# rjagerman/pytorchltr

Hardware: AMD Instinct MI355X
Metric: queries/sec loss fwd+bwd (B=1024, list_len=128) + achieved HBM GB/s (higher is better)
Workload: dtype f32; 1 GPU; c2: Linear(136,1) scorer + hinge loss fwd+bwd, B=1024/GPU, list_len=128, n~U[1,128]; global_batch=1024, list_len=128, features=136, loss=hinge, mode=eager, parallelism=dp1, batches_in_rotation=5, repeats=1, statistic=one timed region of --steps steps after --warmup steps

## Files before the change

### include/ltr_sched.h

```cpp
#ifndef LTR_SCHED_H
#define LTR_SCHED_H

#include "ltr_hip.h"

#ifdef __cplusplus
extern "C" {
#endif

LTR_DEBUG_HOOK int ltr_debug_sched_slots(int B, int G, int cus, int nred, int *group, int *rank);
LTR_DEBUG_HOOK int ltr_debug_lazy_holdback(int packed);

#ifdef __cplusplus
}
#endif

#endif
```

### pytorchltr_amd/_C.py

```python
import ctypes
import os

import torch

_HERE = os.path.dirname(os.path.abspath(__file__))
LIB_PATH = os.environ.get("LTR_HIP_LIB") or os.path.join(_HERE, "csrc", "libltr_hip.so")

HINGE, DCG_HINGE, LOGISTIC, ARP1, ARP2, NDCG1, NDCG2 = range(7)
LABEL_I64, LABEL_F32, LABEL_I32 = 0, 1, 2
ERR_CONFIG = -6
ERR_TIMEOUT = -7
PLAN_NONE, PLAN_REGISTER_TILE, PLAN_CLUSTER, PLAN_GENERAL, PLAN_PARTS = 0, 1, 2, 3, 4

_vp, _i, _f, _sz = ctypes.c_void_p, ctypes.c_int, ctypes.c_float, ctypes.c_size_t

SIGNATURES = {
    "ltr_version": (_i, []),
    "ltr_error_string": (ctypes.c_char_p, [_i]),
    "ltr_max_list_len": (_i, []),
    "ltr_max_list_len_f64": (_i, []),
    "ltr_device_status": (_i, [_i]),
    "ltr_debug_force_timeout": (None, [_i]),
    "ltr_debug_cluster_mode": (None, [_i]),
    "ltr_debug_parts_all": (_i, [_i]),
# ... 53 lines not shown
    "ltr_linear_lazy_rows_reduce_f32": (_i, [_i, _i, _i, _i, _f, _vp, _i, _vp, _vp, _vp, _i, _vp]),
    "ltr_debug_fake_allreduce": (_i, [_vp, _vp, _sz, _i, _i, _vp, _vp]),
    "ltr_mailbox_create": (_i, [_i, _i, _i, _vp, _vp]),
    "ltr_mailbox_connect": (_i, [_vp, _vp]),
    "ltr_mailbox_destroy": (_i, [_vp]),
    "ltr_mailbox_allreduce": (_i, [_vp, _vp, _sz, _i, _i, _vp, _vp]),
    "ltr_debug_mailbox_state": (_i, [_vp, ctypes.c_longlong, ctypes.c_longlong]),
    "ltr_mailbox_set_timeout_ms": (ctypes.c_longlong, [ctypes.c_longlong]),
    "ltr_linear_pairwise_f32": (_i, [_i, _f, _vp, _vp, _vp, _vp, _i, _vp, _vp, _i, _i, _i,
                                     _vp, _vp, _vp, _vp, _vp, _sz, _vp]),
    "ltr_linear_partials_f32": (_i, [_i, _f, _vp, _vp, _vp, _vp, _i, _vp, _i, _i, _i,
                                     _vp, _vp, _vp, _vp]),
    "ltr_linear_reduce_f32": (_i, [_vp, _vp, _i, _i, _vp, _vp, _vp]),
    "ltr_linear_reduce_bcast_f32": (_i, [_vp, _vp, _i, _i, _vp, _vp, _vp]),
    "ltr_linear_reduce_loss_f32": (_i, [_vp, _vp, _vp, _i, _i, _vp, _vp, _vp, _vp]),
    "ltr_linear_reduce_accum_f32": (_i, [_vp, _vp, _vp, _i, _i, _vp, _vp, _vp, _i, _vp]),
    "ltr_linear_scores_f32": (_i, [_vp, _vp, _vp, _vp, _i, _i, _i, _vp, _vp]),
    "ltr_linear_grad_workspace_bytes": (_sz, [_i, _i, _i]),
    "ltr_linear_grad_f32": (_i, [_vp, _vp, _vp, _i, _i, _i, _vp, _vp, _sz, _vp]),
    "ltr_mlp_max_list_len": (_i, [_i]),
    "ltr_mlp_param_count": (_sz, [_i, _i, _i]),
    "ltr_mlp_workspace_bytes": (_sz, [_i, _i, _i, _i]),
    "ltr_mlp_scores_f32": (_i, [_vp, _vp, _vp, _vp, _vp, _vp, _vp, _vp, _i, _i, _i, _i, _i, _vp, _vp]),
    "ltr_mlp_pairwise_f32": (_i, [_i, _f, _vp, _vp, _vp, _vp, _vp, _vp, _vp, _vp, _i, _vp, _vp,
                                  _i, _i, _i, _i, _i, _vp, _vp, _vp, _vp, _vp, _sz, _vp]),
}

EVAL_SIGNATURES = {
    "ltr_eval_workspace_bytes": (_sz, [_i, _i, _vp, _i]),
    "ltr_eval_f32": (_i, [_vp, _vp, _i, _vp, _vp, _i, ctypes.c_uint64, _vp, _i, _i, _vp, _i, _f, _i, _f, _vp, _vp,
                          _sz, _vp]),
}

LISTWISE_LISTNET, LISTWISE_LISTMLE = 0, 1

LISTWISE_SIGNATURES = {
    "ltr_listmle_workspace_bytes": (_sz, [_i, _i]),
    "ltr_listmle_f32": (_i, [_vp, _vp, _i, _vp, _i, _vp, _i, ctypes.c_uint64, _vp, _i, _i, _vp, _vp, _vp, _sz, _vp]),
    "ltr_linear_listwise_plan": (_i, [_i, _i, _i, _i]),
    "ltr_linear_listwise_partials_f32": (_i, [_i, _i, _vp, _vp, _vp, _vp, _i, _vp, _vp, _i, ctypes.c_uint64, _vp, _i, _i, _i,
                                              _vp, _vp, _vp, _vp]),
    "ltr_mlp_listwise_plan": (_i, [_i, _i, _i, _i, _i, _i]),
    "ltr_mlp_listwise_f32": (_i, [_i, _i] + [_vp] * 7 + [_vp, _i, _vp, _vp, _i, ctypes.c_uint64, _vp, _vp]
                             + [_i] * 5 + [_vp] * 5 + [_sz, _vp]),
}

MLP_ROWS_SIGNATURES = {
    "ltr_mlp_rows_scores_f32": (_i, [_vp] * 8 + [_i] * 5 + [_vp, _vp]),
    "ltr_mlp_rows_grad_workspace_bytes": (_sz, [_i, _i, _i, _i, _i]),
    "ltr_mlp_rows_grad_f32": (_i, [_vp] * 9 + [_i] * 5 + [_vp, _vp, _sz, _vp]),
}

MLP_BF16_SIGNATURES = {
    "ltr_mlp_bf16_scores": (_i, [_vp] * 8 + [_i] * 5 + [_vp, _vp]),
    "ltr_mlp_bf16_grad_workspace_bytes": (_sz, [_i, _i, _i, _i, _i]),
    "ltr_mlp_bf16_grad": (_i, [_vp] * 9 + [_i] * 5 + [_vp, _vp, _sz, _vp]),
}

LINEAR_BF16_SIGNATURES = {
    "ltr_linear_scores_bf16": (_i, [_vp, _vp, _vp, _vp, _i, _i, _i, _vp, _vp]),
    "ltr_linear_grad_workspace_bytes_bf16": (_sz, [_i, _i, _i]),
    "ltr_linear_grad_bf16": (_i, [_vp, _vp, _vp, _i, _i, _i, _vp, _vp, _sz, _vp]),
    "ltr_linear_bf16_plan": (_i, [_i, _i, _i, _i]),
    "ltr_linear_partials_bf16": (_i, [_i, _f, _vp, _vp, _vp, _vp, _i, _vp, _i, _i, _i, _vp, _vp, _vp, _vp]),
    "ltr_collate_pad_bf16": (_i, [_vp, _vp, _vp, _vp, _vp, _i, _i, _i, _i, _vp, _vp, _vp, _vp]),
}

MLP_WIDE_SIGNATURES = {
    "ltr_mlp_wide_scores_f32": (_i, [_vp] * 8 + [_i] * 5 + [_vp, _vp]),
    "ltr_mlp_wide_grad_workspace_bytes": (_sz, [_i, _i, _i, _i, _i]),
    "ltr_mlp_wide_grad_f32": (_i, [_vp] * 9 + [_i] * 5 + [_vp, _vp, _sz, _vp]),
}

LONGPAIR_SIGNATURES = {
    "ltr_max_pair_list_len": (_i, []),
    "ltr_long_pair_geometry": (None, [_vp, _vp]),
    "ltr_pairwise_loss_long_workspace_bytes": (_sz, [_i, _i, _i]),
    "ltr_pairwise_loss_long_f32": (_i, [_i, _f, _vp, _vp, _i, _vp, _i, _i, _vp, _vp, _vp, _sz, _vp]),
    "ltr_debug_long_pairs_all": (_i, [_i]),
}

SCHED_SIGNATURES = {
    "ltr_debug_sched_slots": (_i, [_i, _i, _i, _i, _vp, _vp]),
    "ltr_debug_lazy_holdback": (_i, [_i]),
}

_lib = None


class ExtensionMissingError(ImportError):
    pass


class _Library(ctypes.CDLL):

    def __getattr__(self, name):
        try:
            return super().__getattr__(name)
        except AttributeError:
            if name.startswith("ltr_debug_"):
                raise AttributeError(
                    "%s is a test / tuning hook and this libltr_hip.so was built without them (LTR_NO_DEBUG_HOOKS=1); "
                    "rebuild with `python -m pytorchltr_amd.build --force` and the variable unset" % name) from None
            raise


def lib():
    global _lib
    if _lib is None:
        if not os.path.exists(LIB_PATH):
            raise ExtensionMissingError(
                "pytorchltr_amd HIP extension not found at %s; build it with "
                "`python -m pytorchltr_amd.build` (hipcc --offload-arch=gfx950). "
                "There is no CPU fallback." % LIB_PATH)
        handle = _Library(LIB_PATH)
        for name, (restype, argtypes) in (list(SIGNATURES.items()) + list(EVAL_SIGNATURES.items())
                                          + list(LISTWISE_SIGNATURES.items()) + list(LONGPAIR_SIGNATURES.items())
                                          + list(MLP_ROWS_SIGNATURES.items()) + list(MLP_WIDE_SIGNATURES.items())
                                          + list(MLP_BF16_SIGNATURES.items()) + list(LINEAR_BF16_SIGNATURES.items())
                                          + list(SCHED_SIGNATURES.items())):
            if name.startswith("ltr_debug_") and not hasattr(handle, name):
                continue
            fn = getattr(handle, name)
            fn.restype = restype
            fn.argtypes = argtypes
        _lib = handle
    return _lib


def check(rc):
    if rc != 0:
        msg = lib().ltr_error_string(int(rc))
        raise RuntimeError("pytorchltr_amd: %s (code %d)" % (msg.decode() if msg else "?", rc))


def ptr(t):
    return None if t is None else t.data_ptr()


try:
    _raw_stream = torch._C._cuda_getCurrentRawStream
except AttributeError:
    _raw_stream = None


def stream_of(t):
    if _raw_stream is not None:
        return _raw_stream(t.device.index if t.device.index is not None else torch.cuda.current_device())
    return torch.cuda.current_stream(t.device).cuda_stream


class _NullCtx:
    def __enter__(self):
        return self

    def __exit__(self, *exc):
        return False


_NULL = _NullCtx()


def device_ctx(t):
    idx = t.device.index
    if idx is None or idx == torch.cuda.current_device():
        return _NULL
# ... 78 lines not shown
```

### pytorchltr_amd/csrc/ltr_common.inc

```
#pragma once
#include <hip/hip_runtime.h>
#include <hip/hip_ext.h>
#include <stdint.h>
#include <stdio.h>
#include <stdlib.h>
#include <type_traits>

#include "ltr_hip.h"

extern "C" __attribute__((visibility("hidden"))) int *ltr_internal_status_device_ptr(void *stream);
extern "C" __attribute__((visibility("hidden"))) int ltr_internal_status_peek(void);
extern "C" __attribute__((visibility("hidden"))) void ltr_internal_exchange_mark_dirty(void);

namespace {

constexpr int kWave = 64;
constexpr int kMaxListLen = 4096;
constexpr int kSymMaxLen = 1024;
constexpr int kLossSymMaxLen = 2048;
constexpr float kLog2e = 1.4426950408889634f;
constexpr float kLn2 = 0.6931471805599453f;

#define LTR_CLEAR_STALE_ERROR() ((void)hipGetLastError())

// ... 25 lines not shown
    if (dtype == LTR_LABEL_I64)
        stage_rows_t(sy, srow, (const int64_t *)rel + row, L, nb, tid, T);
    else if (dtype == LTR_LABEL_F32)
        stage_rows_t(sy, srow, (const float *)rel + row, L, nb, tid, T);
    else
        stage_rows_t(sy, srow, (const int32_t *)rel + row, L, nb, tid, T);
}

template <typename LabelT>
__device__ __forceinline__ void stage_labels_t(float2 *sy, const LabelT *__restrict__ yrow, int L,
                                               int nb, int tid, int T)
{
    for (int m = tid; m < L; m += T) {
        const float yv = (float)yrow[m];
        if (m < nb) sy[m].y = yv;
    }
}

__device__ __forceinline__ void stage_labels(float2 *sy, const void *rel, int dtype, size_t row,
                                             int L, int nb, int tid, int T)
{
    if (dtype == LTR_LABEL_I64) stage_labels_t(sy, (const int64_t *)rel + row, L, nb, tid, T);
    else if (dtype == LTR_LABEL_F32) stage_labels_t(sy, (const float *)rel + row, L, nb, tid, T);
    else stage_labels_t(sy, (const int32_t *)rel + row, L, nb, tid, T);
}

__device__ __forceinline__ int clamp_n(int64_t n, int L)
{
    return n < 0 ? 0 : (n > (int64_t)L ? L : (int)n);
}

constexpr int kSchedMaxPerCu = 4;
constexpr int kLossSchedMaxPerCu = 16;
constexpr int kSchedLowBits = 3;

struct SchedSlot { int group, rank; };
__host__ __device__ inline int sched_round(int id, int cus, int &r)
{
    int t = 0;
    r = id;
    if (r >= 4 * cus) { r -= 4 * cus; t += 4; }
    if (r >= 2 * cus) { r -= 2 * cus; t += 2; }
    if (r >= cus) { r -= cus; t += 1; }
    return t;
}
__host__ __device__ inline bool sched_quiet(int id, int cus, int nred)
{
    if (nred <= 0 || nred >= cus || id < cus) return false;
    int r;
    sched_round(id, cus, r);
    return r < nred;
}
__host__ __device__ inline SchedSlot sched_slot(int id, int B, int G, int cus, int nred)
{
    int pos = id - nred;
    if (nred > 0 && nred < cus) {
        int r, re;
        const int t = sched_round(id, cus, r);
        const int below = t > 0 ? (t - 1) * nred + (r < nred ? r : nred) : 0;
        if (t > 0 && r < nred) {
            const int te = sched_round(nred + B, cus, re);
            const int Q = te > 0 ? (te - 1) * nred + (re < nred ? re : nred) : 0;
            pos = B - Q + below;
        } else {
            pos -= below;
        }
    }
    const int u = pos >> 3;
    int jp = u / G;
    SchedSlot s;
    s.group = u - jp * G;
    if (cus > 0) {
        const int per = cus / (8 * G);
        if (per >= 2) {
            const int rd = jp / per, base = rd * per;
            const int back = (rd ^ (rd >> 1)) & 1;
            if (back && (base + per) * 8 * G <= B) jp = base + (per - 1 - (jp - base));
        }
    }
    s.rank = jp * 8 + (pos & 7);
    return s;
}

__device__ __forceinline__ int sched_query_sampled(const int64_t *__restrict__ n, int B, int L, int G, int tid,
                                                   int &nb_out, int pos, int round_cus = 0, int nred = 0)
{
    __shared__ int s_sel[2];
    if (tid < 64) {
        const int lane = tid;
        const SchedSlot slot = sched_slot(pos, B, G, round_cus, nred);
        const int gam = slot.group;
        int rho = slot.rank;
        const int id = ((lane >> 3) * G + gam) * 8 + (lane & 7);
        unsigned long long cand = __ballot(id < B);
        const int key = clamp_n(n[min(id, B - 1)], L);
        const bool flat = __ballot(key != __builtin_amdgcn_readfirstlane(key)) == 0ull;
        for (int bt = flat ? -1 : 31 - __builtin_clz(L); bt >= kSchedLowBits; --bt) {
            const unsigned long long m = __ballot(((key >> bt) & 1) != 0) & cand;
            const int c = __popcll(m);
            if (rho < c) cand = m;
            else { rho -= c; cand &= ~m; }
        }
        const int below = __popcll(cand & ((1ull << lane) - 1ull));
        if ((((cand >> lane) & 1ull) != 0ull) && below == rho) { s_sel[0] = id; s_sel[1] = key; }
    }
    __syncthreads();
    nb_out = __builtin_amdgcn_readfirstlane(s_sel[1]);
    return __builtin_amdgcn_readfirstlane(s_sel[0]);
}

template <int CTRL, int ROW_MASK>
__device__ __forceinline__ float dpp_move(float v)
{
    return __int_as_float(__builtin_amdgcn_update_dpp(0, __float_as_int(v), CTRL, ROW_MASK, 0xF, false));
}

__device__ __forceinline__ float quad_sum(float v)
{
    v += dpp_move<0xB1, 0xF>(v);
    v += dpp_move<0x4E, 0xF>(v);
    return v;
}

__device__ __forceinline__ float wave_sum(float v)
{
    v = quad_sum(v);
    v += dpp_move<0x141, 0xF>(v);
    v += dpp_move<0x140, 0xF>(v);
    v += dpp_move<0x142, 0xA>(v);
    v += dpp_move<0x143, 0xC>(v);
    return __int_as_float(__builtin_amdgcn_readlane(__float_as_int(v), 63));
}

__device__ __forceinline__ void lds_barrier()
{
    asm volatile("s_waitcnt lgkmcnt(0)\n\ts_barrier" ::: "memory");
}

__device__ __forceinline__ float block_sum(float v, float *red)
{
    v = wave_sum(v);
    const int nw = blockDim.x >> 6;
    if (nw == 1) return v;
    __syncthreads();
    if ((threadIdx.x & 63) == 0) red[threadIdx.x >> 6] = v;
    __syncthreads();
    float t = 0.f;
    for (int i = 0; i < nw; ++i) t += red[i];
    return t;
}

struct OpAdd { static constexpr float id = 0.f; static __device__ __forceinline__ float f(float a, float b) { return a + b; } };
struct OpMul { static constexpr float id = 1.f; static __device__ __forceinline__ float f(float a, float b) { return a * b; } };
struct OpMin { static constexpr float id = 3.0e38f; static __device__ __forceinline__ float f(float a, float b) { return fminf(a, b); } };

template <typename Op>
__device__ __forceinline__ float block_reduce(float v, float *red)
{
#pragma unroll
    for (int o = 32; o > 0; o >>= 1) v = Op::f(v, __shfl_xor(v, o, kWave));
    const int nw = blockDim.x >> 6;
    if (nw == 1) return v;
    __syncthreads();
    if ((threadIdx.x & 63) == 0) red[threadIdx.x >> 6] = v;
    __syncthreads();
    float t = red[0];
    for (int i = 1; i < nw; ++i) t = Op::f(t, red[i]);
    return t;
}

__device__ __forceinline__ void block_sum2(float &a, float &b, float *red)
{
    a = wave_sum(a);
    b = wave_sum(b);
    const int nw = blockDim.x >> 6;
    if (nw == 1) return;
    __syncthreads();
    if ((threadIdx.x & 63) == 0) { red[2 * (threadIdx.x >> 6)] = a; red[2 * (threadIdx.x >> 6) + 1] = b; }
    __syncthreads();
    float ta = 0.f, tb = 0.f;
    for (int i = 0; i < nw; ++i) { ta += red[2 * i]; tb += red[2 * i + 1]; }
    a = ta;
    b = tb;
}

__device__ __forceinline__ float log2_1p(float e)
{
    const float direct = __builtin_amdgcn_logf(1.0f + e);
    const float series = e * (1.0f - 0.5f * e) * kLog2e;
    return e < 0.0009765625f ? series : direct;
}
// ... 916 lines not shown
```

### pytorchltr_amd/csrc/ltr_linear.inc

```

namespace {

constexpr int kP1Unr = 4;
constexpr int kP3Unr = 4;
constexpr int kLinearThreads = 512;


constexpr int kMbMaxRanks = 16;
struct MailboxDev {
    unsigned long long *peer[kMbMaxRanks];
    int rank, world, count_max, pad;
    long long ticks;
};
constexpr unsigned kLazyPoison = 0x7fc0deadu;

#define LTR_KARG __attribute__((address_space(4)))
struct LinearParams {
    const float *X;
    const float *W;
    const float *bias;
    const void *rel;
    const int64_t *n;
    float *loss;
    float *scores_out;
// ... 317 lines not shown
            float sres = dp ? red[20 + tid] : (red[tid] + red[4 + tid]) + (red[8 + tid] + red[12 + tid]);
            const bool ok = !dp || __float_as_uint(sres) != kLazyPoison;
            if (!ok) sres = __builtin_nanf("");
            p.pend_out[f] = sres;
            float wnew = sres;
            if (f <= F && (!GENERAL || p.pend_W)) {
                float *wp = (f < F) ? p.pend_W + f : p.pend_bias;
                wnew = __builtin_fmaf(-p.pend_lr, sres, wp[0]);
                if (!dp) wp[0] = wnew;
            }
            red[16 + tid] = ok ? wnew : __uint_as_float(kLazyPoison);
        }
    }
    lds_barrier();
    if (p.pend_gran && tid < 4 * kLazyCopies) {
        const int u = tid & 3, copy = tid >> 2;
        const int f = losses ? F + 1 : 4 * bx + u;
        if ((!losses && f <= F) || (losses && u == 0))
            __hip_atomic_store(p.pend_gran + (size_t)copy * p.pend_gstride + f, ((unsigned long long)p.pend_tag << 32) | __float_as_uint(red[16 + u]),
                               __ATOMIC_RELAXED, __HIP_MEMORY_SCOPE_AGENT);
    }
    if (dp && losses && p.pend_gran) {
        lds_barrier();
        if (tid == 0) red[24] = 0.f;
        lds_barrier();
        const unsigned long long *g0 = p.pend_gran;
        bool bad = false;
        for (int g = tid; g < F + 2; g += nt) {
            int spins = 0;
            for (;;) {
                const unsigned long long gv = __hip_atomic_load(g0 + g, __ATOMIC_RELAXED, __HIP_MEMORY_SCOPE_AGENT);
                if ((unsigned)(gv >> 32) == p.pend_tag) { bad = bad || (unsigned)gv == kLazyPoison || p.spin_limit < 0; break; }
                if (++spins > p.spin_limit) { bad = true; break; }
                __builtin_amdgcn_s_sleep(2);
            }
        }
        if (bad) red[24] = 1.f;
        lds_barrier();
        if (red[24] == 0.f)
            for (int g = tid; g <= F; g += nt) {
                const unsigned long long gv = __hip_atomic_load(g0 + g, __ATOMIC_RELAXED, __HIP_MEMORY_SCOPE_AGENT);
                float *wp = (g < F) ? p.pend_W + g : p.pend_bias;
                wp[0] = __uint_as_float((unsigned)gv);
            }
    }
}

__device__ __forceinline__ void linear_lazy_reduce(const LinearParams &p, float *red, const int nt)
{
    if (p.pend_general) linear_lazy_reduce_t<true>(p, red, nt);
    else linear_lazy_reduce_t<false>(p, red, nt);
}

template <int T>
__device__ __forceinline__ void linear_lazy_poll_weights(const LinearParams &p, float *wst, unsigned copy, int tid)
{
    const int F = p.F;
    const unsigned long long *g0 = p.pend_gran + (size_t)(copy & (kLazyCopies - 1)) * p.pend_gstride;
    bool bad = false;
    for (int g = tid; g < F + 2; g += T) {
        unsigned long long gv = 0ull;
        int spins = 0;
        for (;;) {
            gv = __hip_atomic_load(g0 + g, __ATOMIC_RELAXED, __HIP_MEMORY_SCOPE_AGENT);
            if ((unsigned)(gv >> 32) == p.pend_tag && p.spin_limit >= 0) break;
            if (++spins > p.spin_limit) { bad = true; gv = 0x7fc000007fc00000ull; break; }
            __builtin_amdgcn_s_sleep(2);
        }
        wst[g] = __uint_as_float((unsigned)gv);
    }
    if (bad && p.status) __hip_atomic_store(p.status, (int)LTR_ERR_TIMEOUT, __ATOMIC_RELAXED, __HIP_MEMORY_SCOPE_SYSTEM);
}

__global__ void __launch_bounds__(256)
linear_lazy_flush_kernel(LinearParams p)
{
    __shared__ float red[32];
    linear_lazy_reduce(p, red, 256);
}

template <int KIND, int NI, int CT, int TT>
__device__ __forceinline__ void linear_regtile2_body(const LinearParams &p);

template <int KIND, int NI, int CT, int TT>
__global__ void __launch_bounds__(TT, 8) __attribute__((amdgpu_num_sgpr(80)))
linear_regtile2_kernel(LinearParams p)
{
    linear_regtile2_body<KIND, NI, CT, TT>(p);
}

template <int KIND, int NI, int CT, int TT>
__global__ void __launch_bounds__(TT, (TT == 512 && NI < 19 ? kRegtileMinW : 4))
linear_regtile2w_kernel(LinearParams p)
{
    linear_regtile2_body<KIND, NI, CT, TT>(p);
}

template <int KIND, int NI, int CT, int TT>
constexpr auto regtile2_entry()
{
    if constexpr (KIND != LTR_NDCG1 && KIND != LTR_NDCG2 && TT == 512 && NI <= 9) return &linear_regtile2_kernel<KIND, NI, CT, TT>;
    else return &linear_regtile2w_kernel<KIND, NI, CT, TT>;
}

template <int KIND, int NI, int CT, int TT>
__device__ __forceinline__ void linear_regtile2_body(const LinearParams &p)
{
    extern __shared__ __attribute__((aligned(16))) unsigned char smem[];
    constexpr int T = TT;
    const int L = p.L;
    LTR_TRACE_ENTRY();
    const bool lazy = p.pend_B > 0;
    const int qblock = (int)blockIdx.x - (lazy ? p.pend_nred : 0);
    if (lazy && qblock < 0) {
        const LTR_KARG unsigned char *ka = (const LTR_KARG unsigned char *)__builtin_amdgcn_kernarg_segment_ptr();
        asm volatile("" : "+s"(ka));
        LinearParams pr;
#define LTR_KA(field) pr.field = *reinterpret_cast<const LTR_KARG decltype(pr.field) *>(ka + offsetof(LinearParams, field))
        LTR_KA(part); LTR_KA(loss); LTR_KA(F); LTR_KA(pend_B); LTR_KA(pend_g); LTR_KA(pend_nred); LTR_KA(pend_lr); LTR_KA(pend_w);
        LTR_KA(pend_wptr); LTR_KA(pend_wstride); LTR_KA(pend_general); LTR_KA(pend_W); LTR_KA(pend_bias); LTR_KA(pend_out);
        LTR_KA(pend_gran); LTR_KA(pend_gstride); LTR_KA(pend_tag); LTR_KA(status); LTR_KA(spin_limit); LTR_KA(pend_mb);
#undef LTR_KA
        LTR_TRACE_REDUCER(0);
        linear_lazy_reduce(pr, reinterpret_cast<float *>(smem), TT);
        LTR_TRACE_REDUCER(1);
        return;
    }
    const int qhold = lazy ? p.pend_sleep >> 8 : 0;
    if (lazy) {
        const int hold = (qhold && sched_quiet((int)blockIdx.x, p.sched >> 16, p.pend_nred)) ? qhold : (p.pend_sleep & 0xff);
        for (int i = 0; i < hold; ++i) __builtin_amdgcn_s_sleep(8);
    }
    int b, nb;
    if (p.sched) {
        b = sched_query_sampled(p.n, p.B, L, p.sched & 0xffff, (int)threadIdx.x, nb, qhold ? (int)blockIdx.x : qblock, p.sched >> 16,
                                qhold ? p.pend_nred : 0);
    } else {
        b = qblock;
        nb = clamp_n(p.n[b], L);
    }
    const int C = CT > 0 ? CT : (p.F >> 2);
    const int F = C << 2;
    const int R = T / C;
    const int CP = regtile2_cp(C);
    const int L4 = (L + 63) & ~63;
    const int tid = threadIdx.x;
    constexpr int msplit = T >> 6;
    const bool active = tid < R * C;
    const int rq = tid / C;
    const int c = tid - rq * C;
    const int r = active ? rq : (1 << 20);

    const QueryLds q = carve_query_lds<KIND>(smem, L4, msplit);
    size_t off = (loss_lds_bytes(KIND, L4, msplit) + 15) & ~(size_t)15;
    const int Lg = (NI * R + 3) & ~3;
    float *gfin = reinterpret_cast<float *>(smem + off);
    float *pd = gfin + Lg;
    float4 *dred = reinterpret_cast<float4 *>(pd);
    float *bred = reinterpret_cast<float *>(dred + T);
    const size_t row = (size_t)b * L;
    LTR_STAMP2(0);
    LTR_TRACE_PLACEMENT();

    float4 w = make_float4(0.f, 0.f, 0.f, 0.f);
    float bias = 0.f;
    if (!lazy) {
        w = reinterpret_cast<const float4 *>(p.W)[c];
        bias = p.bias ? p.bias[0] : 0.f;
    }
    const uintptr_t xaddr = reinterpret_cast<uintptr_t>(p.X + row * (size_t)F);
    const unsigned xlo = __builtin_amdgcn_readfirstlane((unsigned)xaddr);
    const unsigned xhi = __builtin_amdgcn_readfirstlane((unsigned)(xaddr >> 32));
    const __amdgpu_buffer_rsrc_t rsrc = __builtin_amdgcn_make_buffer_rsrc(
        reinterpret_cast<void *>(((uintptr_t)xhi << 32) | xlo), 0,
        __builtin_amdgcn_readfirstlane(nb * F * 4), 0x00020000);
    const int voff = active ? tid * 16 : 0x7ffffff0;
    const int sweep = R * C * 16;
    float4 x[NI];
#pragma unroll
    for (int i = 0; i < NI; ++i) {
        const ltr_u32x4 v = __builtin_amdgcn_raw_buffer_load_b128(rsrc, voff + i * sweep, 0, 0);
        x[i] = make_float4(__uint_as_float(v.x), __uint_as_float(v.y), __uint_as_float(v.z), __uint_as_float(v.w));
    }
    int ylo = 0, yhi = 0;
    {
        const int wide = (p.rel_dtype == LTR_LABEL_I64) ? 1 : 0;
        const int *rp = reinterpret_cast<const int *>(p.rel) + ((row + (size_t)min(tid, L - 1)) << wide);
        ylo = rp[0];
        yhi = rp[wide];
    }
    if (KIND == LTR_NDCG1 || KIND == LTR_NDCG2)
        for (int m = tid; m < 2 * L4; m += T) q.rank_s[m] = 0;
    LTR_STAMP2(7);

    if (lazy) {
        {
            const size_t pdb = (size_t)4 * L * CP, drb = (size_t)16 * T + 4 * R;
            float *wst = reinterpret_cast<float *>(reinterpret_cast<unsigned char *>(pd) + (((pdb > drb ? pdb : drb) + 15) & ~(size_t)15));
            unsigned xcc;
            asm volatile("s_getreg_b32 %0, hwreg(HW_REG_XCC_ID)" : "=s"(xcc));
            linear_lazy_poll_weights<T>(p, wst, xcc, tid);
            lds_barrier();
            LTR_STAMP2(11);
            w = reinterpret_cast<const float4 *>(wst)[c];
            bias = wst[F];
        }
    }

    {
        float *pdw = pd + (active ? rq : 0) * CP + c;
#pragma unroll
        for (int i = 0; i < NI; ++i)
            if (r < nb - i * R) pdw[i * R * CP] = vdot_pk(x[i], w);
    }
    asm volatile("" : "+v"(ylo), "+v"(yhi));
    if (tid < nb) {
        if (p.rel_dtype != LTR_LABEL_I64) yhi = ylo >> 31;
        const long long y64 = ((long long)yhi << 32) | (unsigned)ylo;
        q.sy[tid].y = (p.rel_dtype == LTR_LABEL_F32) ? __int_as_float(ylo) : (float)y64;
// ... 307 lines not shown
        int owners = 64;
        while (owners < L && owners < T) owners *= 2;
        s.dpt = (L > owners) ? 4 : 1;
        s.msplit = T / owners;
        Ls = (L + 3) & ~3;
        slices = s.msplit;
    }
    s.lds = linear_lds_bytes(kind, Ls, F, slices, s.R);
    while (s.dpt != 0 && s.lds > kLdsBudget && s.msplit > 1) {
        s.msplit /= 2;
        s.lds = linear_lds_bytes(kind, Ls, F, s.msplit, s.R);
    }
    while (s.lds > kLdsBudget && s.R > 1) {
        s.R /= 2;
        s.lds = linear_lds_bytes(kind, Ls, F, s.dpt == 0 ? slices : s.msplit, s.R);
    }
    return s.lds <= kLdsBudget;
}

template <int KIND, int VEC>
int launch_linear_kind(const LinearParams &p, const LinearShape &s, hipStream_t stream)
{
    const dim3 grid((unsigned)p.B), block((unsigned)s.threads);
#define LTR_LAUNCH(D)                                                                           \
    do {                                                                                        \
        constexpr auto entry = linear_pairwise_entry<KIND, D, VEC>();                           \
        LTR_ENSURE_LDS((*entry), s.lds);                                                        \
        hipLaunchKernelGGL(entry, grid, block, s.lds, stream, p);                               \
    } while (0)
    if (s.dpt == 0) LTR_LAUNCH(0);
    else if (s.dpt == 1) LTR_LAUNCH(1);
    else LTR_LAUNCH(4);
#undef LTR_LAUNCH
    return (int)hipGetLastError();
}

template <int VEC>
int launch_linear(int kind, const LinearParams &p, const LinearShape &s, hipStream_t stream)
{
    return with_kind(kind, [&](auto K) { return launch_linear_kind<K, VEC>(p, s, stream); });
}



struct RegtileShape { int ni, threads; size_t lds; };

bool choose_regtile_shape(int kind, int L, int F, RegtileShape &s)
{
    if (F % 4 != 0 || !regtile_sym(L)) return false;
    const int C = F / 4;
    if (C > kRegtileThreads) return false;
    const bool ndcg = (kind == LTR_NDCG1 || kind == LTR_NDCG2);
    const int R = kRegtileThreads / C;
    const int ni = (L + R - 1) / R;
    s.threads = kRegtileThreads;
    if (ni <= 3) s.ni = 3;
    else if (ni <= 5) s.ni = 5;
    else if (ni <= 9) s.ni = 9;
    else if (ni <= 12 && !ndcg) s.ni = 12;
    else {
        const int nsw = (ni <= 19) ? 19 : ((ni <= 24) ? 24 : 0);
        if (nsw == 0) return false;
        s.ni = nsw;
        s.lds = regtile2_lds_bytes(kind, L, F, nsw, kRegtileThreads);
        return s.lds <= 78 * 1024;
    }
    if (ndcg && C <= 256) {
        const int R2 = 256 / C;
        const int ni2 = (L + R2 - 1) / R2;
        const int n2 = ni2 <= 5 ? 5 : (ni2 <= 9 ? 9 : (ni2 <= 12 ? 12 : (ni2 <= 19 ? 19 : 0)));
        if (n2 > 0) {
            const size_t lds256 = regtile2_lds_bytes(kind, L, F, n2, 256);
            if (lds256 <= 40 * 1024) { s.threads = 256; s.ni = n2; s.lds = lds256; return true; }
        }
    }
    s.lds = regtile2_lds_bytes(kind, L, F, s.ni, kRegtileThreads);
    return s.lds <= 64 * 1024;
}

struct KernelEvents { bool armed; hipEvent_t start, stop; };
inline KernelEvents &kernel_events() { static thread_local KernelEvents e = {false, nullptr, nullptr}; return e; }

template <int KIND, int NI, int CT, int TT>
int launch_regtile2_tt(const LinearParams &p, size_t lds, const KernelEvents *ke, hipStream_t stream)
{
    constexpr auto entry = regtile2_entry<KIND, NI, CT, TT>();
    const dim3 grid((unsigned)(p.B + (p.pend_B > 0 ? p.pend_nred : 0)));
    if constexpr (TT == kRegtileThreads && NI >= 19) LTR_ENSURE_LDS((*entry), lds);
    if constexpr (TT == kRegtileThreads && NI <= 9) {
        if (ke) {
            hipExtLaunchKernelGGL(entry, grid, dim3(TT), (unsigned)lds, stream, ke->start, ke->stop, 0, p);
            return (int)hipGetLastError();
        }
    }
    hipLaunchKernelGGL(entry, grid, dim3(TT), lds, stream, p);
    return (int)hipGetLastError();
}

template <int KIND, int NI, int CT>
int launch_regtile2_ni(const LinearParams &p, const RegtileShape &s, const KernelEvents *ke, hipStream_t stream)
{
    constexpr bool ndcg = (KIND == LTR_NDCG1 || KIND == LTR_NDCG2);
    if (s.threads == 256) {
        if constexpr (ndcg && NI != 3 && NI != 24) return launch_regtile2_tt<KIND, NI, CT, 256>(p, s.lds, nullptr, stream);
        else return LTR_ERR_CONFIG;
    }
    if constexpr (ndcg && NI == 12) return LTR_ERR_CONFIG;
    else return launch_regtile2_tt<KIND, NI, CT, kRegtileThreads>(p, s.lds, ke, stream);
}

template <int KIND, int CT>
int launch_regtile2_ct(const LinearParams &p, const RegtileShape &s, hipStream_t stream)
{
    KernelEvents &events = kernel_events();
    const KernelEvents *ke = events.armed ? &events : nullptr;
    events.armed = false;
    switch (s.ni) {
    case 3: return launch_regtile2_ni<KIND, 3, CT>(p, s, ke, stream);
    case 5: return launch_regtile2_ni<KIND, 5, CT>(p, s, ke, stream);
    case 9: return launch_regtile2_ni<KIND, 9, CT>(p, s, ke, stream);
    case 12: return launch_regtile2_ni<KIND, 12, CT>(p, s, ke, stream);
    case 19: return launch_regtile2_ni<KIND, 19, CT>(p, s, ke, stream);
    case 24: return launch_regtile2_ni<KIND, 24, CT>(p, s, ke, stream);
    default: return LTR_ERR_CONFIG;
    }
}

int launch_regtile(int kind, const LinearParams &p, const RegtileShape &s, hipStream_t stream)
{
    return with_kind(kind, [&](auto K) {
        return p.F == 136 ? launch_regtile2_ct<K, 34>(p, s, stream) : launch_regtile2_ct<K, 0>(p, s, stream);
    });
}

}
```

### pytorchltr_amd/csrc/ltr_linear_step.inc

```
namespace {
inline size_t linear_partials_bytes(int B, int F)
{
    const size_t PF = (size_t)partial_pitch(F);
    const size_t split = (B >= kReduceSplitMin && PF / 4 <= 256) ? (size_t)kReduceMaxSplit * (size_t)reduce_scratch_pitch((int)PF) * sizeof(float) : 0;
    return ((((size_t)B * PF * sizeof(float)) + 255) & ~(size_t)255) + split + 256;
}

inline bool step_shape_bad(int B, int L, int F) { return B < 0 || L <= 0 || F <= 0; }
inline bool step_workspace_short(int B, int L, int F, const void *ws, size_t bytes) { return B > 0 && (!ws || bytes < ltr_linear_workspace_bytes(B, L, F)); }

inline bool prefer_cluster()
{
    return !parts_debug_all();
}

struct LinearPlan { int family; RegtileShape rs; ClusterShape cs; PartsShape ps; };

LinearPlan plan_linear(int kind, int B, int L, int F, int vec, bool fast, int labels)
{
    LinearPlan pl;
    pl.family = LTR_PLAN_GENERAL;
    if (vec != 4 || !fast) return pl;
    const bool cluster_first = prefer_cluster();
    if (choose_regtile_shape(kind, L, F, pl.rs)) pl.family = LTR_PLAN_REGISTER_TILE;
    else if (cluster_first && choose_cluster_shape(kind, B, L, F, pl.cs, labels)) pl.family = LTR_PLAN_CLUSTER;
    else if (choose_parts_shape(kind, B, L, F, pl.ps)) pl.family = LTR_PLAN_PARTS;
    else if (!cluster_first && choose_cluster_shape(kind, B, L, F, pl.cs, labels)) pl.family = LTR_PLAN_CLUSTER;
    return pl;
}

constexpr int kLazyHoldPlain = 2, kLazyHold = 0, kLazyHoldQuiet = 8;
inline int &lazy_holdback() { static int v = -1; return v; }
inline bool lazy_quiet_pays(int kind, int B, int F)
{
    return (kind == LTR_HINGE || kind == LTR_DCG_HINGE) && B > 3 * device_cu_count() && F >= 64;
}
}

extern "C" {
LTR_DEBUG_HOOK void ltr_debug_force_timeout(int on) { cluster_force_timeout() = on ? 1 : 0; }
LTR_DEBUG_HOOK void ltr_debug_cluster_mode(int bits) { cluster_debug_mode() = bits; }
LTR_DEBUG_HOOK int ltr_debug_parts_all(int on) { const int old = parts_debug_all(); parts_debug_all() = on ? 1 : 0; return old; }

size_t ltr_linear_workspace_bytes(int B, int L, int F)
{
    if (B <= 0 || F <= 0) return 0;
    size_t bytes = linear_partials_bytes(B, F);
    size_t scratch = 0;
    ClusterShape cs;
    for (int kind = LTR_HINGE; kind <= LTR_NDCG2 && L > 0; ++kind)
        for (int labels = 0; labels <= 1; ++labels)
            if (choose_cluster_shape(kind, B, L, F, cs, labels) && cs.scratch_floats * sizeof(float) > scratch)
                scratch = cs.scratch_floats * sizeof(float);
    return bytes + scratch;
}

int ltr_linear_fused_plan(int kind, int B, int L, int F)
{
    LTR_CLEAR_STALE_ERROR();
    if (kind < LTR_HINGE || kind > LTR_NDCG2 || B <= 0 || L <= 0 || F <= 0) return LTR_PLAN_NONE;
    if (L > kMaxListLen) return LTR_PLAN_NONE;
    return plan_linear(kind, B, L, F, 4, true, -1).family;
}

namespace {
struct LazyRequest {
    int pend_B; float lr; float *W, *bias, *out; unsigned long long *gran; unsigned tag; int part_g, pend_g;
    float scale;
    const float *scale_dev;
    int scale_stride;
    const MailboxDev *mb;
};

inline float pending_weight(float scale, int pend_B) { return scale > 0.f ? scale : 1.0f / (float)pend_B; }

void set_pending_update(LinearParams &p, const LazyRequest &r, int F, bool queries, hipStream_t stream, bool quiet_pays = false)
{
    p.pend_B = r.pend_B; p.pend_g = r.pend_g; p.pend_lr = r.lr; p.pend_w = pending_weight(r.scale, r.pend_B);
    p.pend_mb = r.mb; p.pend_wptr = r.scale_dev; p.pend_wstride = r.scale_stride;
    p.pend_W = r.W; p.pend_bias = r.bias; p.pend_out = r.out;
    p.pend_gran = r.gran; p.pend_tag = r.tag; p.pend_gstride = (F + 2 + 15) & ~15;
    p.pend_nred = (F + 1 + 3) / 4 + 1;
    p.pend_general = (p.pend_mb || p.pend_wptr || !p.pend_W) ? 1 : 0;
    const bool quiet = quiet_pays && p.sched != 0 && p.pend_nred < (p.sched >> 16);
    p.pend_sleep = !queries ? 0 : lazy_holdback() >= 0 ? lazy_holdback() : quiet ? kLazyHoldQuiet << 8 | kLazyHold : kLazyHoldPlain;
    if (queries || r.mb) {
        p.status = status_device_ptr(stream);
        p.spin_limit = cluster_force_timeout() ? -1 : (r.mb ? 0x7fffffff : (1 << 22));
    }
}

int linear_partials_launch(int kind, float sigma, const float *X, const float *W, const float *bias, const void *rel, int rel_dtype,
                           const int64_t *n, int B, int L, int F, float *loss, float *scores_out, float *partials, void *stream,
                           const LazyRequest *lazy)
{
    LTR_CLEAR_STALE_ERROR();
    if (const int rc = check_kind(kind, rel_dtype)) return rc;
    if (step_shape_bad(B, L, F)) return LTR_ERR_SHAPE;
    if (L > kMaxListLen) return LTR_ERR_LIST_TOO_LONG;
    if (B == 0) return LTR_OK;
    if (!X || !W || !rel || !n || !loss || !partials) return LTR_ERR_NULL;
    if (const int st = status_peek()) return st;
    const int vec = (F % 4 == 0 && ((uintptr_t)X % 16 == 0)) ? 4 : 1;
    LinearParams p;
    p.X = X; p.W = W; p.bias = bias; p.rel = rel; p.n = n;
    p.loss = loss; p.scores_out = scores_out; p.part = partials;
    p.B = B; p.L = L; p.F = F; p.sigma = sigma; p.rel_dtype = rel_dtype;
    p.sched = 0; p.rows_r = 0;
    const LinearPlan pl = plan_linear(kind, B, L, F, vec, LTR_TRACE_ALLOW_FAST(scores_out), rel_dtype != LTR_LABEL_F32 ? 1 : 0);
    if (lazy && pl.family != LTR_PLAN_REGISTER_TILE) return LTR_ERR_CONFIG;
    switch (pl.family) {
    case LTR_PLAN_REGISTER_TILE:
        p.msplit = kRegtileThreads / 64;
        p.sched = (L > 64) ? sched_groups(B, kSchedMaxPerCu) : 0;
        if (p.sched) p.sched |= device_cu_count() << 16;
        if (lazy) p.part_g = lazy->part_g;
        p.scores_out = LTR_TRACE_BUFFER(p.scores_out);
        if (lazy && lazy->pend_B > 0) set_pending_update(p, *lazy, F, true, (hipStream_t)stream, lazy_quiet_pays(kind, B, F));
        return launch_regtile(kind, p, pl.rs, (hipStream_t)stream);
    case LTR_PLAN_PARTS:
        p.msplit = 0;
        return launch_parts(kind, p, pl.ps, (hipStream_t)stream);
    case LTR_PLAN_CLUSTER: {
        p.msplit = pl.cs.threads / 64;
        p.sched = (B >= 16) ? (B + 63) / 64 : 0;
        float *scratch = partials + linear_partials_bytes(B, F) / sizeof(float);
        return launch_cluster(kind, p, pl.cs, scratch, (hipStream_t)stream);
    }
    default: break;
    }
    LinearShape s;
    if (!choose_linear_shape(kind, B, L, F, vec, s)) return LTR_ERR_SHAPE;
    p.msplit = s.msplit; p.rows_r = s.R;
    p.sched = sched_groups_for_lists(B, L);
    return (vec == 4) ? launch_linear<4>(kind, p, s, (hipStream_t)stream)
                      : launch_linear<1>(kind, p, s, (hipStream_t)stream);
}
}

int ltr_linear_partials_f32(int kind, float sigma, const float *X, const float *W,
                            const float *bias, const void *rel, int rel_dtype,
                            const int64_t *n, int B, int L, int F, float *loss,
                            float *scores_out, float *partials, void *stream)
{
    return linear_partials_launch(kind, sigma, X, W, bias, rel, rel_dtype, n, B, L, F, loss, scores_out, partials, stream, nullptr);
}

LTR_DEBUG_HOOK int ltr_debug_sched_slots(int B, int G, int cus, int nred, int *group, int *rank)
{
    if (B <= 0 || G <= 0 || cus < 0 || nred < 0) return LTR_ERR_SHAPE;
    if (nred > 0 && nred < cus && (long long)B + nred >= 8ll * cus) return LTR_ERR_SHAPE;
    if (!group || !rank) return LTR_ERR_NULL;
    for (int i = 0; i < B; ++i) {
        const SchedSlot s = sched_slot(nred + i, B, G, cus, nred);
        group[i] = s.group;
        rank[i] = s.rank;
    }
    return LTR_OK;
}

#ifdef LTR_TRACE
int ltr_debug_trace_buffer(void *buf) { trace_buffer() = (float *)buf; return LTR_OK; }
#endif

LTR_DEBUG_HOOK int ltr_debug_kernel_events(void *start, void *stop)
{
    KernelEvents &ke = kernel_events();
    ke.start = (hipEvent_t)start; ke.stop = (hipEvent_t)stop;
    ke.armed = start != nullptr && stop != nullptr;
    return LTR_OK;
}

LTR_DEBUG_HOOK int ltr_debug_stream_probe_f32(const float *X, const int64_t *n, int B, int L, int F, float *out, void *stream)
{
    LTR_CLEAR_STALE_ERROR();
    if (B <= 0 || L <= 0 || F <= 0 || F % 4 != 0) return LTR_ERR_SHAPE;
    if (!X || !n || !out) return LTR_ERR_NULL;
    const long long vecs = (long long)L * (F / 4);
    const dim3 grid((unsigned)B);
    hipStream_t st = (hipStream_t)stream;
#define LTR_PROBE(NI_, TT_) hipLaunchKernelGGL((stream_probe_kernel<NI_, TT_>), grid, dim3(TT_), 0, st, X, n, L, F, out)
    if (vecs <= 3 * 512) LTR_PROBE(3, 512);
    else if (vecs <= 5 * 512) LTR_PROBE(5, 512);
    else if (vecs <= 9 * 512) LTR_PROBE(9, 512);
    else if (vecs <= 12 * 512) LTR_PROBE(12, 512);
    else if (vecs <= 19 * 512) LTR_PROBE(19, 512);
    else return LTR_ERR_SHAPE;
#undef LTR_PROBE
    return (int)hipGetLastError();
}

int ltr_linear_reduce_accum_f32(const float *partials, const float *grad_out, const float *loss,
                                int B, int F, float *dW, float *db, float *loss_sum, int accumulate,
                                void *stream)
{
    LTR_CLEAR_STALE_ERROR();
    if (B < 0 || F <= 0) return LTR_ERR_SHAPE;
    if (!dW || !db) return LTR_ERR_NULL;
    if (B > 0 && !partials) return LTR_ERR_NULL;
    if ((loss_sum != nullptr) && B > 0 && !loss) return LTR_ERR_NULL;
    if (const int st = status_peek()) return st;
    return launch_linear_reduce((hipStream_t)stream, partials, grad_out, B > 0 ? 1.0f / (float)B : 0.f, 1, B, F, dW, db, loss, loss_sum,
                                accumulate ? 1 : 0, nullptr, nullptr, 0.f);
}

int ltr_linear_reduce_bcast_f32(const float *partials, const float *scale, int B, int F, float *dW, float *db, void *stream)
{
    LTR_CLEAR_STALE_ERROR();
    if (B < 0 || F <= 0) return LTR_ERR_SHAPE;
    if (!dW || !db || !scale) return LTR_ERR_NULL;
    if (B > 0 && !partials) return LTR_ERR_NULL;
    if (const int st = status_peek()) return st;
    return launch_linear_reduce((hipStream_t)stream, partials, scale, 0.f, 0, B, F, dW, db, nullptr, nullptr, 0, nullptr, nullptr, 0.f);
}

int ltr_linear_reduce_loss_f32(const float *partials, const float *grad_out, const float *loss,
                               int B, int F, float *dW, float *db, float *loss_sum, void *stream)
{
    LTR_CLEAR_STALE_ERROR();
    return ltr_linear_reduce_accum_f32(partials, grad_out, loss, B, F, dW, db, loss_sum, 0, stream);
}

int ltr_linear_reduce_f32(const float *partials, const float *grad_out, int B, int F, float *dW,
                          float *db, void *stream)
{
    LTR_CLEAR_STALE_ERROR();
    return ltr_linear_reduce_loss_f32(partials, grad_out, nullptr, B, F, dW, db, nullptr, stream);
}

int ltr_linear_step_f32(int kind, float sigma, const float *X, const float *W, const float *bias,
                        const void *rel, int rel_dtype, const int64_t *n, const float *grad_out,
                        int B, int L, int F, float *loss, float *bucket, int accumulate,
                        void *workspace, size_t workspace_bytes, void *overlap, int slot, void *stream)
{
    LTR_CLEAR_STALE_ERROR();
    if (step_shape_bad(B, L, F)) return LTR_ERR_SHAPE;
    if (!bucket) return LTR_ERR_NULL;
    if (step_workspace_short(B, L, F, workspace, workspace_bytes)) return LTR_ERR_WORKSPACE;
    LtrOverlap *o = reinterpret_cast<LtrOverlap *>(overlap);
    if (o && o->depth > 0 && (slot < 0 || slot >= o->depth)) return LTR_ERR_CONFIG;
// ... 64 lines not shown
```

Baseline: 80.71 million queries/s.

## Precompute per-block schedule slots on host and pass table via kernel arguments

Each block's schedule slot (group, rank, quiet flag) was computed on device by sched_slot arithmetic. It is now precomputed on the host, cached, and passed as a 16-bit-per-block table appended to the kernel argument block, so each block reads its entry from the kernarg segment. This removes per-block scalar integer math (divisions, reversal logic) from the kernel prologue, at the cost of a larger kernarg copy per launch and a cache lookup under a mutex. The lazy holdback constants also change: plain hold goes from 2 to 3 sleep iterations, and non-quiet blocks beside quiet ones now hold 1-2 instead of 0.

Result: no change. 80.97 million queries/s, median of 6 (+0.3%).

```diff
diff --git a/include/ltr_sched.h b/include/ltr_sched.h
--- a/include/ltr_sched.h
+++ b/include/ltr_sched.h
@@ -8,6 +8,7 @@
 #endif
 
 LTR_DEBUG_HOOK int ltr_debug_sched_slots(int B, int G, int cus, int nred, int *group, int *rank);
+LTR_DEBUG_HOOK int ltr_debug_sched_table(int B, int G, int cus, int nred, int quiet, unsigned short *entries, int *sizes);
 LTR_DEBUG_HOOK int ltr_debug_lazy_holdback(int packed);
 
 #ifdef __cplusplus
diff --git a/pytorchltr_amd/_C.py b/pytorchltr_amd/_C.py
--- a/pytorchltr_amd/_C.py
+++ b/pytorchltr_amd/_C.py
@@ -159,6 +159,7 @@
 
 SCHED_SIGNATURES = {
     "ltr_debug_sched_slots": (_i, [_i, _i, _i, _i, _vp, _vp]),
+    "ltr_debug_sched_table": (_i, [_i, _i, _i, _i, _i, _vp, _vp]),
     "ltr_debug_lazy_holdback": (_i, [_i]),
 }
 
diff --git a/pytorchltr_amd/csrc/ltr_common.inc b/pytorchltr_amd/csrc/ltr_common.inc
--- a/pytorchltr_amd/csrc/ltr_common.inc
+++ b/pytorchltr_amd/csrc/ltr_common.inc
@@ -131,13 +131,25 @@
     return s;
 }
 
-__device__ __forceinline__ int sched_query_sampled(const int64_t *__restrict__ n, int B, int L, int G, int tid,
-                                                   int &nb_out, int pos, int round_cus = 0, int nred = 0)
+constexpr int kSchedTableCus = 304;
+constexpr int kSchedTableReducers = 176;
+constexpr int kSchedTableEntries = kSchedMaxPerCu * kSchedTableCus + kSchedTableReducers;
+struct alignas(8) SchedTable { unsigned short e[kSchedTableEntries]; };
+constexpr unsigned short kSchedEntryReducer = 0x7fffu;
+__host__ __device__ inline unsigned short sched_entry_pack(SchedSlot s, bool quiet)
+{
+    return (unsigned short)((s.group & 0xff) | (s.rank & 0x7f) << 8 | (quiet ? 0x8000 : 0));
+}
+__host__ __device__ inline SchedSlot sched_entry_slot(unsigned e) { SchedSlot s; s.group = (int)(e & 0xff); s.rank = (int)(e >> 8 & 0x7f); return s; }
+__host__ __device__ inline bool sched_entry_quiet(unsigned e) { return (e & 0x8000u) != 0; }
+
+template <class SlotFn>
+__device__ __forceinline__ int sched_query_select(const int64_t *__restrict__ n, int B, int L, int G, int tid, int &nb_out, SlotFn slot_of)
 {
     __shared__ int s_sel[2];
     if (tid < 64) {
         const int lane = tid;
-        const SchedSlot slot = sched_slot(pos, B, G, round_cus, nred);
+        const SchedSlot slot = slot_of();
         const int gam = slot.group;
         int rho = slot.rank;
         const int id = ((lane >> 3) * G + gam) * 8 + (lane & 7);
@@ -156,6 +168,12 @@
     __syncthreads();
     nb_out = __builtin_amdgcn_readfirstlane(s_sel[1]);
     return __builtin_amdgcn_readfirstlane(s_sel[0]);
+}
+
+__device__ __forceinline__ int sched_query_sampled(const int64_t *__restrict__ n, int B, int L, int G, int tid,
+                                                   int &nb_out, int pos, int round_cus = 0, int nred = 0)
+{
+    return sched_query_select(n, B, L, G, tid, nb_out, [=]() { return sched_slot(pos, B, G, round_cus, nred); });
 }
 
 template <int CTRL, int ROW_MASK>
diff --git a/pytorchltr_amd/csrc/ltr_linear.inc b/pytorchltr_amd/csrc/ltr_linear.inc
--- a/pytorchltr_amd/csrc/ltr_linear.inc
+++ b/pytorchltr_amd/csrc/ltr_linear.inc
@@ -423,16 +423,33 @@
 template <int KIND, int NI, int CT, int TT>
 __device__ __forceinline__ void linear_regtile2_body(const LinearParams &p);
 
+constexpr size_t kSchedTableOffset = sizeof(LinearParams);
+static_assert(sizeof(LinearParams) % alignof(SchedTable) == 0, "the table stands right behind LinearParams");
+static_assert(kSchedTableOffset + sizeof(SchedTable) <= 4096, "LinearParams and the schedule table must fit the 4 KB argument block");
+
+__device__ __forceinline__ unsigned sched_table_entry()
+{
+    const LTR_KARG unsigned char *ka = (const LTR_KARG unsigned char *)__builtin_amdgcn_kernarg_segment_ptr();
+    const unsigned id = min((unsigned)blockIdx.x, (unsigned)(kSchedTableEntries - 1));
+    const unsigned w = *reinterpret_cast<const LTR_KARG unsigned *>(ka + kSchedTableOffset + ((id >> 1) << 2));
+    return (w >> ((id & 1u) << 4)) & 0xffffu;
+}
+
+__device__ __forceinline__ int sched_query_table(const int64_t *__restrict__ n, int B, int L, int G, int tid, int &nb_out, unsigned entry)
+{
+    return sched_query_select(n, B, L, G, tid, nb_out, [=]() { return sched_entry_slot(entry); });
+}
+
 template <int KIND, int NI, int CT, int TT>
 __global__ void __launch_bounds__(TT, 8) __attribute__((amdgpu_num_sgpr(80)))
-linear_regtile2_kernel(LinearParams p)
+linear_regtile2_kernel(LinearParams p, SchedTable)
 {
     linear_regtile2_body<KIND, NI, CT, TT>(p);
 }
 
 template <int KIND, int NI, int CT, int TT>
 __global__ void __launch_bounds__(TT, (TT == 512 && NI < 19 ? kRegtileMinW : 4))
-linear_regtile2w_kernel(LinearParams p)
+linear_regtile2w_kernel(LinearParams p, SchedTable)
 {
     linear_regtile2_body<KIND, NI, CT, TT>(p);
 }
@@ -451,6 +468,8 @@
     constexpr int T = TT;
     const int L = p.L;
     LTR_TRACE_ENTRY();
+    const unsigned slot = sched_table_entry();
+    asm volatile("" :: "s"(slot), "s"(p.n), "s"(p.B), "s"(p.L), "s"(p.sched), "s"(p.pend_sleep));
     const bool lazy = p.pend_B > 0;
     const int qblock = (int)blockIdx.x - (lazy ? p.pend_nred : 0);
     if (lazy && qblock < 0) {
@@ -467,15 +486,13 @@
         LTR_TRACE_REDUCER(1);
         return;
     }
-    const int qhold = lazy ? p.pend_sleep >> 8 : 0;
     if (lazy) {
-        const int hold = (qhold && sched_quiet((int)blockIdx.x, p.sched >> 16, p.pend_nred)) ? qhold : (p.pend_sleep & 0xff);
+        const int hold = sched_entry_quiet(slot) ? p.pend_sleep >> 8 : (p.pend_sleep & 0xff);
         for (int i = 0; i < hold; ++i) __builtin_amdgcn_s_sleep(8);
     }
     int b, nb;
     if (p.sched) {
-        b = sched_query_sampled(p.n, p.B, L, p.sched & 0xffff, (int)threadIdx.x, nb, qhold ? (int)blockIdx.x : qblock, p.sched >> 16,
-                                qhold ? p.pend_nred : 0);
+        b = sched_query_table(p.n, p.B, L, p.sched & 0xffff, (int)threadIdx.x, nb, slot);
     } else {
         b = qblock;
         nb = clamp_n(p.n[b], L);
@@ -949,54 +966,54 @@
 inline KernelEvents &kernel_events() { static thread_local KernelEvents e = {false, nullptr, nullptr}; return e; }
 
 template <int KIND, int NI, int CT, int TT>
-int launch_regtile2_tt(const LinearParams &p, size_t lds, const KernelEvents *ke, hipStream_t stream)
+int launch_regtile2_tt(const LinearParams &p, const SchedTable &tab, size_t lds, const KernelEvents *ke, hipStream_t stream)
 {
     constexpr auto entry = regtile2_entry<KIND, NI, CT, TT>();
     const dim3 grid((unsigned)(p.B + (p.pend_B > 0 ? p.pend_nred : 0)));
     if constexpr (TT == kRegtileThreads && NI >= 19) LTR_ENSURE_LDS((*entry), lds);
     if constexpr (TT == kRegtileThreads && NI <= 9) {
         if (ke) {
-            hipExtLaunchKernelGGL(entry, grid, dim3(TT), (unsigned)lds, stream, ke->start, ke->stop, 0, p);
+            hipExtLaunchKernelGGL(entry, grid, dim3(TT), (unsigned)lds, stream, ke->start, ke->stop, 0, p, tab);
             return (int)hipGetLastError();
         }
     }
-    hipLaunchKernelGGL(entry, grid, dim3(TT), lds, stream, p);
+    hipLaunchKernelGGL(entry, grid, dim3(TT), lds, stream, p, tab);
     return (int)hipGetLastError();
 }
 
 template <int KIND, int NI, int CT>
-int launch_regtile2_ni(const LinearParams &p, const RegtileShape &s, const KernelEvents *ke, hipStream_t stream)
+int launch_regtile2_ni(const LinearParams &p, const SchedTable &tab, const RegtileShape &s, const KernelEvents *ke, hipStream_t stream)
 {
     constexpr bool ndcg = (KIND == LTR_NDCG1 || KIND == LTR_NDCG2);
     if (s.threads == 256) {
-        if constexpr (ndcg && NI != 3 && NI != 24) return launch_regtile2_tt<KIND, NI, CT, 256>(p, s.lds, nullptr, stream);
+        if constexpr (ndcg && NI != 3 && NI != 24) return launch_regtile2_tt<KIND, NI, CT, 256>(p, tab, s.lds, nullptr, stream);
         else return LTR_ERR_CONFIG;
     }
     if constexpr (ndcg && NI == 12) return LTR_ERR_CONFIG;
-    else return launch_regtile2_tt<KIND, NI, CT, kRegtileThreads>(p, s.lds, ke, stream);
+    else return launch_regtile2_tt<KIND, NI, CT, kRegtileThreads>(p, tab, s.lds, ke, stream);
 }
 
 template <int KIND, int CT>
-int launch_regtile2_ct(const LinearParams &p, const RegtileShape &s, hipStream_t stream)
+int launch_regtile2_ct(const LinearParams &p, const SchedTable &tab, const RegtileShape &s, hipStream_t stream)
 {
     KernelEvents &events = kernel_events();
     const KernelEvents *ke = events.armed ? &events : nullptr;
     events.armed = false;
     switch (s.ni) {
-    case 3: return launch_regtile2_ni<KIND, 3, CT>(p, s, ke, stream);
-    case 5: return launch_regtile2_ni<KIND, 5, CT>(p, s, ke, stream);
-    case 9: return launch_regtile2_ni<KIND, 9, CT>(p, s, ke, stream);
-    case 12: return launch_regtile2_ni<KIND, 12, CT>(p, s, ke, stream);
-    case 19: return launch_regtile2_ni<KIND, 19, CT>(p, s, ke, stream);
-    case 24: return launch_regtile2_ni<KIND, 24, CT>(p, s, ke, stream);
+    case 3: return launch_regtile2_ni<KIND, 3, CT>(p, tab, s, ke, stream);
+    case 5: return launch_regtile2_ni<KIND, 5, CT>(p, tab, s, ke, stream);
+    case 9: return launch_regtile2_ni<KIND, 9, CT>(p, tab, s, ke, stream);
+    case 12: return launch_regtile2_ni<KIND, 12, CT>(p, tab, s, ke, stream);
+    case 19: return launch_regtile2_ni<KIND, 19, CT>(p, tab, s, ke, stream);
+    case 24: return launch_regtile2_ni<KIND, 24, CT>(p, tab, s, ke, stream);
     default: return LTR_ERR_CONFIG;
     }
 }
 
-int launch_regtile(int kind, const LinearParams &p, const RegtileShape &s, hipStream_t stream)
+int launch_regtile(int kind, const LinearParams &p, const SchedTable &tab, const RegtileShape &s, hipStream_t stream)
 {
     return with_kind(kind, [&](auto K) {
-        return p.F == 136 ? launch_regtile2_ct<K, 34>(p, s, stream) : launch_regtile2_ct<K, 0>(p, s, stream);
+        return p.F == 136 ? launch_regtile2_ct<K, 34>(p, tab, s, stream) : launch_regtile2_ct<K, 0>(p, tab, s, stream);
     });
 }
 
diff --git a/pytorchltr_amd/csrc/ltr_linear_step.inc b/pytorchltr_amd/csrc/ltr_linear_step.inc
--- a/pytorchltr_amd/csrc/ltr_linear_step.inc
+++ b/pytorchltr_amd/csrc/ltr_linear_step.inc
@@ -29,7 +29,8 @@
     return pl;
 }
 
-constexpr int kLazyHoldPlain = 2, kLazyHold = 0, kLazyHoldQuiet = 8;
+constexpr int kLazyHoldPlain = 3, kLazyHoldQuiet = 8;
+inline int lazy_hold_beside_quiet(int F) { return F >= 128 ? 2 : 1; }
 inline int &lazy_holdback() { static int v = -1; return v; }
 inline bool lazy_quiet_pays(int kind, int B, int F)
 {
@@ -72,6 +73,8 @@
     const MailboxDev *mb;
 };
 
+inline int lazy_reducers(int F) { return (F + 1 + 3) / 4 + 1; }
+
 inline float pending_weight(float scale, int pend_B) { return scale > 0.f ? scale : 1.0f / (float)pend_B; }
 
 void set_pending_update(LinearParams &p, const LazyRequest &r, int F, bool queries, hipStream_t stream, bool quiet_pays = false)
@@ -80,14 +83,44 @@
     p.pend_mb = r.mb; p.pend_wptr = r.scale_dev; p.pend_wstride = r.scale_stride;
     p.pend_W = r.W; p.pend_bias = r.bias; p.pend_out = r.out;
     p.pend_gran = r.gran; p.pend_tag = r.tag; p.pend_gstride = (F + 2 + 15) & ~15;
-    p.pend_nred = (F + 1 + 3) / 4 + 1;
+    p.pend_nred = lazy_reducers(F);
     p.pend_general = (p.pend_mb || p.pend_wptr || !p.pend_W) ? 1 : 0;
     const bool quiet = quiet_pays && p.sched != 0 && p.pend_nred < (p.sched >> 16);
-    p.pend_sleep = !queries ? 0 : lazy_holdback() >= 0 ? lazy_holdback() : quiet ? kLazyHoldQuiet << 8 | kLazyHold : kLazyHoldPlain;
+    p.pend_sleep = !queries ? 0 : lazy_holdback() >= 0 ? lazy_holdback() : quiet ? kLazyHoldQuiet << 8 | lazy_hold_beside_quiet(F) : kLazyHoldPlain;
     if (queries || r.mb) {
         p.status = status_device_ptr(stream);
         p.spin_limit = cluster_force_timeout() ? -1 : (r.mb ? 0x7fffffff : (1 << 22));
     }
+}
+
+bool sched_table_fill(int B, int G, int cus, int nred, bool quiet, SchedTable &t)
+{
+    if (B <= 0 || G <= 0 || G > 256 || cus < 0 || nred < 0 || (long long)B + nred > kSchedTableEntries) return false;
+    if (quiet && nred > 0 && nred < cus && (long long)B + nred >= 8ll * cus) return false;
+    memset(&t, 0, sizeof(t));
+    for (int id = 0; id < nred; ++id) t.e[id] = kSchedEntryReducer;
+    for (int id = nred; id < nred + B; ++id)
+        t.e[id] = quiet ? sched_entry_pack(sched_slot(id, B, G, cus, nred), sched_quiet(id, cus, nred))
+                        : sched_entry_pack(sched_slot(id - nred, B, G, cus, 0), false);
+    return true;
+}
+
+struct SchedTableKey { int B, G, cus, nred, quiet; };
+struct SchedTableCache { std::mutex m; int next = 0; SchedTableKey key[4] = {}; SchedTable tab[4]; };
+bool sched_table_get(int B, int G, int cus, int nred, bool quiet, SchedTable &out)
+{
+    static SchedTableCache C;
+    const SchedTableKey k{B, G, cus, nred, quiet ? 1 : 0};
+    std::lock_guard<std::mutex> lock(C.m);
+    for (int i = 0; i < 4; ++i)
+        if (memcmp(&C.key[i], &k, sizeof(k)) == 0) { out = C.tab[i]; return true; }
+    const int i = C.next;
+    C.key[i] = SchedTableKey{};
+    if (!sched_table_fill(B, G, cus, nred, quiet, C.tab[i])) return false;
+    C.key[i] = k;
+    C.next = (i + 1) & 3;
+    out = C.tab[i];
+    return true;
 }
 
 int linear_partials_launch(int kind, float sigma, const float *X, const float *W, const float *bias, const void *rel, int rel_dtype,
@@ -110,14 +143,20 @@
     const LinearPlan pl = plan_linear(kind, B, L, F, vec, LTR_TRACE_ALLOW_FAST(scores_out), rel_dtype != LTR_LABEL_F32 ? 1 : 0);
     if (lazy && pl.family != LTR_PLAN_REGISTER_TILE) return LTR_ERR_CONFIG;
     switch (pl.family) {
-    case LTR_PLAN_REGISTER_TILE:
+    case LTR_PLAN_REGISTER_TILE: {
         p.msplit = kRegtileThreads / 64;
-        p.sched = (L > 64) ? sched_groups(B, kSchedMaxPerCu) : 0;
+        const bool pending = lazy && lazy->pend_B > 0;
+        const int nred = pending ? lazy_reducers(F) : 0;
+        p.sched = (L > 64 && B + nred <= kSchedTableEntries) ? sched_groups(B, kSchedMaxPerCu) : 0;
         if (p.sched) p.sched |= device_cu_count() << 16;
         if (lazy) p.part_g = lazy->part_g;
         p.scores_out = LTR_TRACE_BUFFER(p.scores_out);
-        if (lazy && lazy->pend_B > 0) set_pending_update(p, *lazy, F, true, (hipStream_t)stream, lazy_quiet_pays(kind, B, F));
-        return launch_regtile(kind, p, pl.rs, (hipStream_t)stream);
+        if (pending) set_pending_update(p, *lazy, F, true, (hipStream_t)stream, lazy_quiet_pays(kind, B, F));
+        SchedTable tab;
+        if (!p.sched) memset(&tab, 0, sizeof(tab));
+        else if (!sched_table_get(B, p.sched & 0xffff, p.sched >> 16, nred, pending && (p.pend_sleep >> 8) != 0, tab)) return LTR_ERR_CONFIG;
+        return launch_regtile(kind, p, tab, pl.rs, (hipStream_t)stream);
+    }
     case LTR_PLAN_PARTS:
         p.msplit = 0;
         return launch_parts(kind, p, pl.ps, (hipStream_t)stream);
@@ -156,6 +195,16 @@
         group[i] = s.group;
         rank[i] = s.rank;
     }
+    return LTR_OK;
+}
+
+LTR_DEBUG_HOOK int ltr_debug_sched_table(int B, int G, int cus, int nred, int quiet, unsigned short *entries, int *sizes)
+{
+    if (sizes) { sizes[0] = (int)sizeof(LinearParams); sizes[1] = (int)sizeof(SchedTable); sizes[2] = kSchedTableEntries; }
+    if (!entries) return sizes ? LTR_OK : LTR_ERR_NULL;
+    SchedTable t;
+    if (!sched_table_get(B, G, cus, nred, quiet != 0, t)) return LTR_ERR_SHAPE;
+    memcpy(entries, t.e, sizeof(unsigned short) * (size_t)(nred + B));
     return LTR_OK;
 }
 
```
